# rubendhz/houdini-gsplat-renderer

Hardware: AMD Instinct MI355X
Metric: frames/sec at 1920x1080 + achieved HBM GB/s (blend kernel) (higher is better)
Workload: dtype f32

## Files before the change

houdini-gsplat-renderer_amd/csrc/gsr_device.h:

```cpp
#pragma once
#ifdef GSR_KPROF
#include <hip/hip_runtime.h>
__device__ unsigned long long g_kprof[8][16];
__device__ unsigned int g_kprof_blk[5][2][8192];
#define KPROF_BLK_BEGIN const unsigned long long kp0_ = wall_clock64();
#define KPROF_BLK_END(k, items) { if (threadIdx.x == 0 && blockIdx.x < 8192) { g_kprof_blk[k][0][blockIdx.x] = (unsigned int)(wall_clock64() - kp0_); g_kprof_blk[k][1][blockIdx.x] = (unsigned int)(items); } }
#define KPROF(k, i) { if (blockIdx.x == 0 && threadIdx.x == 0) g_kprof[k][i] = wall_clock64(); }
#define KPROFB(k, i, blk) { if (blockIdx.x == (blk) && threadIdx.x == 0) g_kprof[k][i] = wall_clock64(); }
#else
#define KPROF(k, i)
#define KPROFB(k, i, blk)
#define KPROF_BLK_BEGIN
#define KPROF_BLK_END(k, items)
#endif

#include <hip/hip_runtime.h>
#include <stdint.h>
#include "gsr_mailbox.h"

#define GSR_TILE_PX 16
#define GSR_WAVE 64

struct __attribute__((aligned(16))) GsrRecord {
    float cx, cy, hx, hy;
    float a1x, a1y, b1x, b1y;
    float r, g, b, la;
};
static_assert(sizeof(GsrRecord) == 48, "record layout");
#define GSR_KAPPA 1.2011224087864498f
#define GSR_QLIM  (2.0f * GSR_KAPPA)

struct GsrFrame {
    float ov[12];
    float pr[16];
    float vw[12];
    float ob[9];
    float io[9];
    float cam[3];
    float origin[3];
    float limx, limy;
    float sigma_vo2;
    float focal;
    float W, H;
    int32_t width, height;
    int32_t sh_order;
    int32_t tiles_x;
    int32_t tiles_y;
    int32_t shard_index, shard_count;
    int32_t shard_rpb;
    int32_t shard_first;
    int32_t local_tiles_y;
    int32_t super;
    int32_t super_shift;
    int32_t stiles_x, stiles_y;
    int32_t flags;
    uint32_t key_min, key_max;
    int32_t pyr_off[6];
    int32_t cull_dilate;
    int32_t rect_shift;
    int32_t phase;
    uint32_t idx_mask;
    float zq0, zqs;
};
typedef const GsrFrame __attribute__((address_space(4)))* GsrFrameArg;
__device__ __forceinline__ GsrFrameArg gsr_frame_arg(unsigned kernarg_off)
{
    static_assert(alignof(GsrFrame) == 4 && sizeof(GsrFrame) % 4 == 0, "the frame is a run of dwords");
    return (GsrFrameArg)((const char __attribute__((address_space(4)))*)__builtin_amdgcn_kernarg_segment_ptr() + kernarg_off);
}
__device__ __forceinline__ GsrFrame gsr_frame_fetch(GsrFrameArg p)
{
    asm volatile("" : "+s"(p));
    GsrFrame f;
    __builtin_memcpy(&f, p, sizeof(GsrFrame));
    return f;
}
#define GSR_ZQ_SHIFT 23
#define GSR_ZQ_MAX 511.0f
#define GSR_SLAB_BINS 1024
#define GSR_FLAG_NO_ALPHA_RADIUS 1
#define GSR_FLAG_NO_SAT          2
#define GSR_FLAG_FULL_KEYS       4
#define GSR_FLAG_LAZY_NO_PREFIX  8
#define GSR_FLAG_CULL_ROUNDS    16
#define GSR_FLAG_NO_DEPTH_CLASS 32
#define GSR_FLAG_NO_ZCODES      64

#ifndef BK_BUCKETS
#define BK_BUCKETS 1024
#endif
#ifndef BK_CAP
#define BK_CAP 8192
#endif
#define BK_STRIDE 64

__device__ __forceinline__ float gsr_fma(float a, float b, float c) { return __builtin_fmaf(a, b, c); }

__device__ __forceinline__ uint32_t gsr_zq(float zw, float z0, float zs)
{
    const float t = __builtin_fminf(__builtin_fmaxf((zw - z0) * zs, 0.0f), GSR_ZQ_MAX);
    return (uint32_t)t;
}

__device__ __forceinline__ float gsr_h2f(uint32_t bits16)
{
    _Float16 h = __builtin_bit_cast(_Float16, (uint16_t)bits16);
    return (float)h;
}

#define GSR_FMT_RGBA32F 0
#define GSR_FMT_RGBA16F 1
#define GSR_FMT_RGBA8   2
__host__ __device__ __forceinline__ int gsr_format_pixel_bytes(int format)
{
    return format == GSR_FMT_RGBA32F ? 16 : format == GSR_FMT_RGBA16F ? 8 : format == GSR_FMT_RGBA8 ? 4 : 0;
}
__host__ __device__ __forceinline__ uint32_t gsr_channel_half(float x)
{
    const _Float16 h = (_Float16)x;
    return (uint32_t)__builtin_bit_cast(uint16_t, h);
}
__host__ __device__ __forceinline__ uint32_t gsr_channel_unorm8(float x)
{
    float c = x > 0.0f ? x : 0.0f;
    c = c < 1.0f ? c : 1.0f;
    return (uint32_t)__builtin_fmaf(c, 255.0f, 0.5f);
}
__host__ __device__ __forceinline__ uint2 gsr_pack_rgba16f(float r, float g, float b, float a)
{
    uint2 o;
    o.x = gsr_channel_half(r) | (gsr_channel_half(g) << 16);
    o.y = gsr_channel_half(b) | (gsr_channel_half(a) << 16);
    return o;
}
__host__ __device__ __forceinline__ uint32_t gsr_pack_rgba8(float r, float g, float b, float a)
{
    return gsr_channel_unorm8(r) | (gsr_channel_unorm8(g) << 8) | (gsr_channel_unorm8(b) << 16) | (gsr_channel_unorm8(a) << 24);
}
__device__ __forceinline__ void gsr_store_packed(void* __restrict__ target, int format, size_t p, float r, float g, float b, float a)
{
    if (format == GSR_FMT_RGBA16F) reinterpret_cast<uint2*>(target)[p] = gsr_pack_rgba16f(r, g, b, a);
    else reinterpret_cast<uint32_t*>(target)[p] = gsr_pack_rgba8(r, g, b, a);
}

__host__ __device__ __forceinline__ float gsr_resolve_depth_pixel(float zsum, float cov, float cov_min)
{
    return cov >= cov_min ? __builtin_fminf(zsum / cov, 1.0f) : 1.0f;
}

#define GSR_BGK_COLOUR 1
#define GSR_BGK_IMAGE  2
__host__ __device__ __forceinline__ float4 gsr_composite_over_pixel(float4 s, float4 b)
{
    const float k = 1.0f - b.w;
    return make_float4(__builtin_fmaf(k, s.x, b.x), __builtin_fmaf(k, s.y, b.y), __builtin_fmaf(k, s.z, b.z), __builtin_fmaf(k, s.w, b.w));
}
__host__ __device__ __forceinline__ float4 gsr_background_pixel(const void* __restrict__ image, int format, size_t p)
{
    if (format == GSR_FMT_RGBA32F) return reinterpret_cast<const float4*>(image)[p];
    if (format == GSR_FMT_RGBA16F) {
        const uint2 v = reinterpret_cast<const uint2*>(image)[p];
        return make_float4((float)__builtin_bit_cast(_Float16, (uint16_t)(v.x & 0xffffu)), (float)__builtin_bit_cast(_Float16, (uint16_t)(v.x >> 16)),
                           (float)__builtin_bit_cast(_Float16, (uint16_t)(v.y & 0xffffu)), (float)__builtin_bit_cast(_Float16, (uint16_t)(v.y >> 16)));
    }
// ... 158 lines not shown
```

houdini-gsplat-renderer_amd/csrc/k_binning.h:

```cpp
#pragma once
#include "gsr_device.h"
#include "k_sort.h"

#define BN_THREADS 256
#ifndef BN_ITEMS
#define BN_ITEMS 4
#endif
#define BN_TILE (BN_THREADS * BN_ITEMS)
#define BN_WAVE_ITEMS (BN_TILE / 4)
#define BN_BINS 256

#define BN_BIG 8

__device__ __forceinline__ uint32_t bn_tile_mask(uint32_t rc, int sx, int sy, int shift)
{
    const int x0 = rc & 255, y0 = (rc >> 8) & 255, x1 = (rc >> 16) & 255, y1 = rc >> 24;
    const int e = (1 << shift) - 1;
    const int c0 = max(x0 - (sx << shift), 0), c1 = min(x1 - (sx << shift), e);
    const int r0 = max(y0 - (sy << shift), 0), r1 = min(y1 - (sy << shift), e);
    const uint32_t cols = ((2u << c1) - 1u) & ~((1u << c0) - 1u), rows = ((2u << r1) - 1u) & ~((1u << r0) - 1u);
    return cols | (rows << 16);
}

template <typename F>
__device__ __forceinline__ void bn_for_each_super(uint32_t rc, int shift, const GsrShard& sh, int stiles_x, int row_lo, int row_hi, F&& fn)
{
    const int x0 = rc & 255, y0 = (rc >> 8) & 255, x1 = (rc >> 16) & 255, y1 = rc >> 24;
    if (x1 < x0 || y1 < y0) return;
    const int sx0 = x0 >> shift, sx1 = x1 >> shift;
    for (int sy = max(y0 >> shift, row_lo); sy <= min(y1 >> shift, row_hi); ++sy) {
        if (sh.count > 1 || sh.rpb > 0) {
            const int lo = max(y0, sy << shift), hi = min(y1, ((sy + 1) << shift) - 1);
            if (gsr_owned_rect_rows(lo, hi, sh) == 0) continue;
        }
        const uint32_t rowkey = (uint32_t)sy * (uint32_t)stiles_x;
        for (int sx = sx0; sx <= sx1; ++sx) fn(rowkey + (uint32_t)sx, sx, sy);
    }
}

#ifndef BN_SPLIT_TILES
#define BN_SPLIT_TILES 16
#endif
struct BnPart { uint32_t tile; int row_lo, row_hi; };
__device__ __forceinline__ uint32_t bn_items(uint32_t nb, int rows) { const uint32_t hs = nb < (uint32_t)BN_SPLIT_TILES ? nb : (uint32_t)BN_SPLIT_TILES; return nb + hs * (uint32_t)(rows - 1); }
__device__ __forceinline__ BnPart bn_part(uint32_t v, uint32_t nb, int rows)
{
    const uint32_t hs = nb < (uint32_t)BN_SPLIT_TILES ? nb : (uint32_t)BN_SPLIT_TILES;
    if (v < hs * (uint32_t)rows) { const uint32_t t = v / (uint32_t)rows; const int r = (int)(v - t * (uint32_t)rows); return BnPart{t, r, r}; }
    return BnPart{hs + rs_tile_of_block(v - hs * (uint32_t)rows, nb - hs, true), 0, 0x7fffffff};
}

template <typename F>
__device__ __forceinline__ void bn_group_pairs(uint2 v, int shift, const GsrShard& sh, int stiles_x, int row_lo, int row_hi, F&& fn)
{
    const int lane = threadIdx.x & 63;
    const uint32_t rc = v.y;
    const int x0 = rc & 255, y0 = (rc >> 8) & 255, x1 = rc >> 16 & 255, y1 = rc >> 24;
    const bool some = x1 >= x0 && y1 >= y0;
    const int ya = max(y0 >> shift, row_lo), yb = min(y1 >> shift, row_hi);
    const int area = (some && yb >= ya) ? ((x1 >> shift) - (x0 >> shift) + 1) * (yb - ya + 1) : 0;
#ifndef BN_MANY
#define BN_MANY 6
#endif
#ifndef BN_BIG_MANY
#define BN_BIG_MANY 32
#endif
    const int thr = __builtin_popcountll(__ballot(area > BN_BIG)) > BN_MANY ? BN_BIG_MANY : BN_BIG;
    const bool big = area > thr;
    if (!big) bn_for_each_super(rc, shift, sh, stiles_x, row_lo, row_hi, [&](uint32_t d, int sx, int sy) { fn(lane, v, d, sx, sy); });
    unsigned long long bigs = __ballot(big);
    while (bigs) {
        const int L = __builtin_ctzll(bigs);
        bigs &= bigs - 1ull;
        const uint2 vL = make_uint2((uint32_t)__shfl((int)v.x, L, 64), (uint32_t)__shfl((int)v.y, L, 64));
        const uint32_t r = vL.y;
        const int X0 = r & 255, Y0 = (r >> 8) & 255, X1 = (r >> 16) & 255, Y1 = r >> 24;
        const int sx0 = X0 >> shift, sy0 = max(Y0 >> shift, row_lo);
        const int w = (X1 >> shift) - sx0 + 1, h = min(Y1 >> shift, row_hi) - sy0 + 1;
        auto cell = [&](int ry, int cx) __attribute__((always_inline)) {
            const int sy = sy0 + ry, sx = sx0 + cx;
            if (sh.count > 1 || sh.rpb > 0) {
                const int lo = max(Y0, sy << shift), hi = min(Y1, ((sy + 1) << shift) - 1);
                if (gsr_owned_rect_rows(lo, hi, sh) == 0) return;
            }
            const uint32_t dd = (uint32_t)sy * (uint32_t)stiles_x + (uint32_t)sx;
            fn(L, vL, dd, sx, sy);
        };
        if (w <= 64) {
            const int cb = w > 1 ? 32 - __builtin_clz((unsigned)(w - 1)) : 0;
            const int cx = lane & ((1 << cb) - 1), rstep = 64 >> cb;
            if (cx < w)
                for (int ry = lane >> cb; ry < h; ry += rstep) cell(ry, cx);
        } else {
            for (int t = lane; t < w * h; t += 64) { const int ry = t / w; cell(ry, t - ry * w); }
        }
    }
}

template <int ITEMS>
__global__ void __launch_bounds__(BN_THREADS)
k_bin_count(const uint2* __restrict__ sorted, const uint32_t* __restrict__ n_dev, int shift, GsrShard sh,
            int stiles_x, int stiles_y, uint32_t* __restrict__ hist, uint32_t nblk)
{
    constexpr uint32_t TILE = BN_THREADS * ITEMS;
    __shared__ uint32_t h[4][BN_BINS];
    KPROF_BLK_BEGIN
    const int wave = threadIdx.x >> 6;
    const uint32_t n = *n_dev;
    const uint32_t nb = (n + TILE - 1) / TILE;
    const uint32_t nv = bn_items(nb, stiles_y);
    for (uint32_t wi = blockIdx.x; wi < nv; wi += gridDim.x) {
        for (int b = threadIdx.x; b < 4 * BN_BINS; b += BN_THREADS) (&h[0][0])[b] = 0;
        __syncthreads();
        const BnPart part = bn_part(wi, nb, stiles_y);
        const uint32_t tile = part.tile;
        {
            const uint32_t base = tile * TILE;
#pragma unroll
            for (int k = 0; k < ITEMS; ++k) {
                const uint32_t i = base + k * BN_THREADS + threadIdx.x;
                const uint2 v = (i < n) ? sorted[i] : make_uint2(0u, GSR_RECT_EMPTY);
                bn_group_pairs(v, shift, sh, stiles_x, part.row_lo, part.row_hi,
                               [&](int, uint2, uint32_t d, int, int) { if (d < (uint32_t)BN_BINS) atomicAdd(&h[wave][d], 1u); });
            }
        }
        __syncthreads();
        const int b_lo = part.row_lo * stiles_x, b_hi = part.row_hi >= stiles_y - 1 ? BN_BINS : (part.row_hi + 1) * stiles_x;
        for (int b = b_lo + (int)threadIdx.x; b < b_hi; b += BN_THREADS)
            hist[(size_t)b * nblk + tile] = h[0][b] + h[1][b] + h[2][b] + h[3][b];
        __syncthreads();
    }
    KPROF_BLK_END(3, n < TILE ? n : TILE)
}

struct GsrRangeArgs {
    const uint32_t* totals;
    int32_t n_super;
    int32_t *sstart, *send;
    volatile unsigned long long* host_total;
    uint32_t ticket;
    unsigned long long max_pairs;
    uint32_t* redo_count;
    const uint32_t* lazy_hint;
    const uint32_t* n_sorted;
    const uint32_t* k1_counts;
    const uint32_t* sorted_keys;
    const uint32_t* depth_active;
};
__device__ __forceinline__ uint32_t bn_ranges(const GsrRangeArgs& a, bool publish, uint32_t* s_wave , unsigned long long* s_sum )
{
    if (publish && threadIdx.x == 0) {
        *a.redo_count = 0u;
        const uint32_t ns = *a.n_sorted;
        a.host_total[1] = ((unsigned long long)ns << 32) | (unsigned long long)(*a.lazy_hint & GSR_HINT_VERDICTS) |
                          (a.k1_counts[2] ? (unsigned long long)GSR_HINT_SORT_GAVE_UP : 0ull) |
                          ((a.depth_active && *a.depth_active) ? (unsigned long long)GSR_HINT_DEPTH_COVERED : 0ull);
        a.host_total[2] = (unsigned long long)a.k1_counts[1];
        a.host_total[3] = ns ? ((unsigned long long)a.sorted_keys[ns - 1u] << 32) | (unsigned long long)a.sorted_keys[0] : 0ull;
    }
    const uint32_t v = ((int)threadIdx.x < a.n_super) ? a.totals[threadIdx.x] : 0u;
    unsigned long long w = v;
#pragma unroll
    for (int d = 32; d > 0; d >>= 1) w += __shfl_down(w, d, 64);
    if ((threadIdx.x & 63) == 0) s_sum[threadIdx.x >> 6] = w;
    uint32_t tot;
    const uint32_t ex = block_excl_scan_256(v, s_wave, &tot);
    const bool too_many = s_sum[0] + s_sum[1] + s_sum[2] + s_sum[3] > a.max_pairs;
    if (publish) {
        if ((int)threadIdx.x < a.n_super) {
            a.sstart[threadIdx.x] = too_many ? 0 : (int32_t)ex;
            a.send[threadIdx.x] = too_many ? 0 : (int32_t)(ex + v);
        }
        if (threadIdx.x == 0) { *a.host_total = ((unsigned long long)a.ticket << 32) | (too_many ? (unsigned long long)GSR_MB_TOO_MANY_PAIRS : (unsigned long long)tot); __threadfence_system(); }
    }
    return too_many ? 0u : ex;
}
__global__ void __launch_bounds__(BN_BINS)
k_bin_ranges(GsrRangeArgs a)
{
    __shared__ uint32_t s_wave[4];
    __shared__ unsigned long long s_sum[4];
    (void)bn_ranges(a, true, s_wave, s_sum);
}

template <int ITEMS, bool ZQ>
__global__ void __launch_bounds__(BN_THREADS)
k_bin_place(const uint2* __restrict__ sorted, const uint32_t* __restrict__ n_dev, int shift, GsrShard sh,
            int stiles_x, int ns, const uint32_t* __restrict__ offs, const int32_t* __restrict__ sstart,
            uint32_t nblk, uint32_t cap, uint2* __restrict__ out, GsrRangeArgs ranges,
            const float* __restrict__ zwin, float zq0, float zqs)
{
    static_assert(BN_THREADS == BN_BINS, "one thread per super-tile in the range scan");
    constexpr uint32_t TILE = BN_THREADS * ITEMS;
    constexpr int NG = 4 * ITEMS;
    KPROF(0, 0)
    KPROF_BLK_BEGIN
    extern __shared__ unsigned long long bn_lds[];
    __shared__ uint32_t s_start[BN_BINS];
    __shared__ uint32_t s_rwave[4];
    __shared__ unsigned long long s_rsum[4];
    const uint32_t n = *n_dev;
    const uint32_t nb = (n + TILE - 1) / TILE;
    const bool publisher = ranges.totals && blockIdx.x == gridDim.x - 1u;
    const uint32_t workers = ranges.totals ? gridDim.x - 1u : gridDim.x;
    if (!publisher && blockIdx.x >= bn_items(nb, stiles_x > 0 ? (ns + stiles_x - 1) / stiles_x : 1)) return;
    if (ranges.totals) {
        s_start[threadIdx.x] = bn_ranges(ranges, publisher, s_rwave, s_rsum);
        if (publisher) return;
    } else {
        s_start[threadIdx.x] = ((int)threadIdx.x < ns) ? (uint32_t)sstart[threadIdx.x] : 0u;
    }
    __syncthreads();
    KPROF(0, 1)
    const int wave = threadIdx.x >> 6;
    unsigned long long* lmask = bn_lds;
    uint32_t* gpre = reinterpret_cast<uint32_t*>(bn_lds + (size_t)NG * ns);
    const int stiles_y = stiles_x > 0 ? (ns + stiles_x - 1) / stiles_x : 1;
    const uint32_t nv = bn_items(nb, stiles_y);
    for (uint32_t wi = blockIdx.x; wi < nv; wi += workers) {
    const BnPart part = bn_part(wi, nb, stiles_y);
    const uint32_t tile = part.tile;
    const uint32_t first = tile * TILE;
    KPROF(0, 2)
    for (int b = threadIdx.x; b < NG * ns; b += BN_THREADS) lmask[b] = 0ull;
    __syncthreads();
    KPROF(0, 3)
    uint2 v[ITEMS];
#pragma unroll
    for (int k = 0; k < ITEMS; ++k) {
        const int grp = k * 4 + wave;
        const uint32_t i = first + (uint32_t)grp * 64u + (threadIdx.x & 63u);
        v[k] = (i < n) ? sorted[i] : make_uint2(0u, GSR_RECT_EMPTY);
        if (ZQ && i < n) v[k].x |= gsr_zq(zwin[v[k].x], zq0, zqs) << GSR_ZQ_SHIFT;
        bn_group_pairs(v[k], shift, sh, stiles_x, part.row_lo, part.row_hi,
                       [&](int L, uint2, uint32_t d, int, int) { if (d < (uint32_t)ns) atomicOr(&lmask[grp * ns + d], 1ull << L); });
    }
    __syncthreads();
    KPROF(0, 4)
    for (int d = threadIdx.x; d < ns; d += BN_THREADS) {
        uint32_t p = s_start[d] + offs[(size_t)d * nblk + tile];
#pragma unroll
        for (int grp = 0; grp < NG; ++grp) { gpre[grp * ns + d] = p; p += (uint32_t)__builtin_popcountll(lmask[grp * ns + d]); }
    }
    __syncthreads();
    KPROF(0, 6)
#pragma unroll
    for (int k = 0; k < ITEMS; ++k) {
        const int grp = k * 4 + wave;
        bn_group_pairs(v[k], shift, sh, stiles_x, part.row_lo, part.row_hi, [&](int L, uint2 vL, uint32_t d, int sx, int sy) {
            if (d >= (uint32_t)ns) return;
            const uint32_t pos = gpre[grp * ns + d] + (uint32_t)__builtin_popcountll(lmask[grp * ns + d] & ((1ull << L) - 1ull));
            if (pos < cap) out[pos] = make_uint2(vL.x, bn_tile_mask(vL.y, sx, sy, shift));
        });
    }
    KPROF(0, 7)
    __syncthreads();
    }
    KPROF_BLK_END(0, n < TILE ? n : TILE)
}

template <typename PIX>
__global__ void __launch_bounds__(256)
k_stitch_bands(const PIX* __restrict__ gathered, int count, int rpb, int band_rows, int width, int height,
               PIX* __restrict__ out)
{
    const size_t p = (size_t)blockIdx.x * 256u + threadIdx.x;
    if (p >= (size_t)width * height) return;
    const int x = (int)(p % width), y = (int)(p / width);
    const int trow = y >> 4;
    const int g = rpb > 0 ? trow / rpb : trow % count, lrow = rpb > 0 ? trow - g * rpb : trow / count;
    const int by = lrow * GSR_TILE_PX + (y & 15);
    out[p] = gathered[((size_t)g * band_rows + by) * width + x];
}
```

houdini-gsplat-renderer_amd/csrc/k_sort.h:

```cpp
#pragma once
#include "gsr_device.h"

#define RS_THREADS 256
#ifndef RS_ITEMS
#define RS_ITEMS 12
#endif
static_assert(RS_ITEMS % 4 == 0, "k_radix_hist reads uint4");
#ifndef RS_ITEMS_MID
#define RS_ITEMS_MID 4
#endif
#define RS_TILE (RS_THREADS * RS_ITEMS)
#define RS_WAVE_ITEMS (RS_TILE / 4)
#ifndef RS_XCD_DEPTH
#define RS_XCD_DEPTH 1
#endif
#ifndef RS_XCD_BIN
#define RS_XCD_BIN 0
#endif

__device__ __forceinline__ uint32_t rs_tile_of_block(uint32_t b, uint32_t nb, bool contig)
{
    if (!contig) return b;
    const uint32_t q = nb >> 3, r = nb & 7u, x = b & 7u, i = b >> 3;
    return x * q + (x < r ? x : r) + i;
// ... 183 lines not shown
    V v_[ITEMS];
    const unsigned long long lt_mask = (1ull << lane) - 1ull;
    uint32_t gc[WAVE_BLOCKS];
    const uint32_t g_first = (tile_base + (uint32_t)wave * WAVE_ITEMS) / RS_SRC_BLOCK;
    const uint32_t g_tot = GATHER ? rs_gather_counts(src_cnt, g_first, (n + RS_SRC_BLOCK - 1) / RS_SRC_BLOCK, gc) : 0u;
#pragma unroll
    for (int r = 0; r < ITEMS; ++r) {
        const uint32_t li = wave * WAVE_ITEMS + r * 64 + lane;
        bool valid = li < nvalid;
        uint32_t key = 0xffffffffu;
        V val{};
        if (GATHER) {
            if ((uint32_t)(r * 64) >= g_tot) { k_[r] = key; v_[r] = val; meta[r] = 0xffffffffu; continue; }
            const uint32_t q = (uint32_t)(r * 64 + lane);
            valid = q < g_tot;
            if (valid) {
                const uint32_t slot = rs_gather_slot(q, g_first, gc);
                key = keys_in[slot];
                val = vals_in[slot];
            }
        } else if (valid) {
            key = keys_in[tile_base + li];
            val = vals_in[tile_base + li];
        }
        const uint32_t d = rs_digit<CLAMP>(key, shift, lo, MASK);
        unsigned long long m = __ballot(valid);
#pragma unroll
        for (int b = 0; b < DBITS; ++b) {
            const bool bit = (d >> b) & 1u;
            const unsigned long long bal = __ballot(bit);
            m &= bit ? bal : ~bal;
        }
        const uint32_t rank = (uint32_t)__builtin_popcountll(m & lt_mask);
        const uint32_t cnt = (uint32_t)__builtin_popcountll(m);
        uint32_t prev = 0;
        if (valid && rank == 0) {
            prev = wc[wave][d];
            wc[wave][d] = prev + cnt;
        }
        const int leader = m ? __builtin_ctzll(m) : 0;
        prev = __shfl(prev, leader, 64);
        k_[r] = key; v_[r] = val;
        meta[r] = valid ? (d | ((prev + rank) << DBITS)) : 0xffffffffu;
    }
    __syncthreads();
    {
        uint32_t tot_d[PER], tsum = 0;
#pragma unroll
        for (int k = 0; k < PER; ++k) {
            const int d = threadIdx.x * PER + k;
            const uint32_t c0 = wc[0][d], c1 = wc[1][d], c2 = wc[2][d], c3 = wc[3][d];
            wc[0][d] = 0; wc[1][d] = c0; wc[2][d] = c0 + c1; wc[3][d] = c0 + c1 + c2;
            tot_d[k] = c0 + c1 + c2 + c3;
            tsum += tot_d[k];
        }
        uint32_t tot;
        uint32_t ex = block_excl_scan_256(tsum, s_wave, &tot);
        if (threadIdx.x == 0) s_tile_items = tot;
#pragma unroll
        for (int k = 0; k < PER; ++k) {
            const int d = threadIdx.x * PER + k;
            dbase[d] = ex;
            gadj[d] = gadj[d] + offs[(size_t)d * nblk + tile] - ex;
            ex += tot_d[k];
        }
    }
    __syncthreads();
#pragma unroll
    for (int r = 0; r < ITEMS; ++r) {
        if (meta[r] == 0xffffffffu) continue;
        const uint32_t d = meta[r] & MASK;
        const uint32_t lp = dbase[d] + wc[wave][d] + (meta[r] >> DBITS);
        skeys[lp] = k_[r];
        svals[lp] = v_[r];
    }
    __syncthreads();
    const uint32_t tile_items = s_tile_items;
#pragma unroll
    for (int r = 0; r < ITEMS; ++r) {
        const uint32_t j = r * RS_THREADS + threadIdx.x;
        if (j < tile_items) {
            const uint32_t key = skeys[j];
            const uint32_t pos = gadj[rs_digit<CLAMP>(key, shift, lo, MASK)] + j;
            keys_out[pos] = key;
            vals_out[pos] = svals[j];
        }
    }
}

__global__ void __launch_bounds__(256)
k_pos_keys(const float4* __restrict__ geoA, uint32_t n, float cx, float cy, float cz, uint32_t key_min, uint32_t key_max,
           uint32_t* __restrict__ keys, uint32_t* __restrict__ vals)
{
    const uint32_t i = blockIdx.x * 256u + threadIdx.x;
    if (i >= n) return;
    const float4 a = geoA[i];
    const float dx = a.x - cx, dy = a.y - cy, dz = a.z - cz;
    const float d2 = __builtin_fmaf(dz, dz, __builtin_fmaf(dy, dy, dx * dx));
    uint32_t b = __builtin_bit_cast(uint32_t, d2);
    b = b < key_min ? key_min : (b > key_max ? key_max : b);
    keys[i] = b - key_min;
    vals[i] = i;
}
__global__ void __launch_bounds__(1024)
k_scan_counts(const uint32_t* __restrict__ cnt, const uint32_t* __restrict__ slots_dev, uint32_t* __restrict__ pre, uint32_t* __restrict__ n_out)
{
    __shared__ uint32_t s_w[16];
    __shared__ uint32_t s_carry;
    const uint32_t m = *slots_dev / (uint32_t)RS_SRC_BLOCK;
    const int lane = threadIdx.x & 63, wave = threadIdx.x >> 6;
    if (threadIdx.x == 0) s_carry = 0u;
    __syncthreads();
    for (uint32_t base = 0; base < m; base += 1024u) {
        const uint32_t j = base + threadIdx.x;
        const uint32_t v = j < m ? cnt[j] : 0u;
        uint32_t x = v;
#pragma unroll
        for (int d = 1; d < 64; d <<= 1) { const uint32_t y = __shfl_up(x, d, 64); if (lane >= d) x += y; }
        if (lane == 63) s_w[wave] = x;
        __syncthreads();
        uint32_t wbase = 0;
        for (int w = 0; w < wave; ++w) wbase += s_w[w];
        const uint32_t carry = s_carry;
        if (j < m) pre[j] = carry + wbase + x - v;
        __syncthreads();
        if (threadIdx.x == 1023) s_carry = carry + wbase + x;
        __syncthreads();
    }
    if (threadIdx.x == 0) *n_out = s_carry;
}
template <typename V>
__global__ void __launch_bounds__(RS_SRC_BLOCK)
k_compact_blocks(const uint32_t* __restrict__ keys_in, const V* __restrict__ vals_in, const uint32_t* __restrict__ cnt, const uint32_t* __restrict__ pre,
                 const uint32_t* __restrict__ slots_dev, uint32_t* __restrict__ keys_out, V* __restrict__ vals_out)
{
    const uint32_t k = blockIdx.x;
    if (k * (uint32_t)RS_SRC_BLOCK >= *slots_dev) return;
    if (threadIdx.x < cnt[k]) {
        const uint32_t src = k * (uint32_t)RS_SRC_BLOCK + threadIdx.x, dst = pre[k] + threadIdx.x;
        keys_out[dst] = keys_in[src];
        vals_out[dst] = vals_in[src];
    }
}

#define RL_THREADS 256
#ifndef RL_ITEMS
#define RL_ITEMS 8
#endif
#define RL_CHUNK (RL_THREADS * RL_ITEMS)
#define RL_WAVE_ITEMS (RL_CHUNK / 4)
#define RL_BINS 256
static_assert(BK_CAP >= RL_CHUNK, "a bucket's region holds at least one chunk");
#define RL_MAX_RUN 64

__device__ __forceinline__ uint32_t rl_id(uint32_t v) { return v; }
__device__ __forceinline__ uint32_t rl_id(uint2 v) { return v.x; }

template <typename V, bool GATHER>
__global__ void __launch_bounds__(RS_THREADS)
k_bucket_scatter(const uint32_t* __restrict__ keys_in, const V* __restrict__ vals_in, uint32_t n_host, const uint32_t* __restrict__ n_dev,
                 int shift, uint32_t lo, const uint32_t* __restrict__ src_cnt ,
                 uint32_t* __restrict__ gcnt , uint32_t* __restrict__ kout, V* __restrict__ vout,
                 uint32_t* __restrict__ n_out , uint32_t* __restrict__ failed)
{
    __shared__ uint32_t h[BK_BUCKETS];
    __shared__ uint32_t s_wave[4];
    const int lane = threadIdx.x & 63, wave = threadIdx.x >> 6;
    KPROF(1, 0)
    KPROF_BLK_BEGIN
    const uint32_t n = n_dev ? *n_dev : n_host;
    const uint32_t nb = (n + RS_TILE - 1) / RS_TILE;
    if (blockIdx.x >= nb) return;
    for (int b = threadIdx.x; b < BK_BUCKETS; b += RS_THREADS) h[b] = 0;
    __syncthreads();
    KPROF(1, 1)
    const uint32_t tile_base = blockIdx.x * RS_TILE;
    const uint32_t nvalid = (n - tile_base < RS_TILE) ? (n - tile_base) : RS_TILE;
    uint32_t k_[RS_ITEMS], meta[RS_ITEMS];
    static_assert(BK_BUCKETS <= 4096 && RS_TILE < (1 << 20), "meta packing");
    V v_[RS_ITEMS];
    uint32_t gc[RS_WAVE_BLOCKS];
    const uint32_t g_first = (tile_base + (uint32_t)wave * RS_WAVE_ITEMS) / RS_SRC_BLOCK;
    const uint32_t g_tot = GATHER ? rs_gather_counts(src_cnt, g_first, (n + RS_SRC_BLOCK - 1) / RS_SRC_BLOCK, gc) : 0u;
    uint32_t mine = 0;
#pragma unroll
    for (int r = 0; r < RS_ITEMS; ++r) {
        const uint32_t li = wave * RS_WAVE_ITEMS + r * 64 + lane;
        bool valid = li < nvalid;
        uint32_t key = 0u;
        V val{};
        if (GATHER) {
            const uint32_t q = (uint32_t)(r * 64 + lane);
            valid = q < g_tot;
            if (valid) { const uint32_t slot = rs_gather_slot(q, g_first, gc); key = keys_in[slot]; val = vals_in[slot]; }
        } else if (valid) {
            key = keys_in[tile_base + li]; val = vals_in[tile_base + li];
        }
        k_[r] = key; v_[r] = val; meta[r] = 0xffffffffu;
        if (valid) {
            const uint32_t d = rs_digit<true>(key, shift, lo, BK_BUCKETS - 1);
            meta[r] = d | (atomicAdd(&h[d], 1u) << 12);
            ++mine;
        }
    }
    __syncthreads();
    KPROF(1, 2)
    for (int d = threadIdx.x; d < BK_BUCKETS; d += RS_THREADS) {
        const uint32_t c = h[d];
        h[d] = c ? atomicAdd(&gcnt[(size_t)d * BK_STRIDE], c) : 0u;
    }
    if (n_out) {
        uint32_t tot;
        (void)block_excl_scan_256(mine, s_wave, &tot);
        if (threadIdx.x == 0 && tot) atomicAdd(n_out, tot);
    }
    __syncthreads();
    KPROF(1, 3)
#pragma unroll
    for (int r = 0; r < RS_ITEMS; ++r) {
        if (meta[r] == 0xffffffffu) continue;
        const uint32_t d = meta[r] & 4095u, p = h[d] + (meta[r] >> 12);
        if (p < (uint32_t)BK_CAP) { kout[(size_t)d * BK_CAP + p] = k_[r]; vout[(size_t)d * BK_CAP + p] = v_[r]; }
        else if (failed) *failed = 1u;
    }
    KPROF(1, 4)
    KPROF_BLK_END(1, mine)
}

template <typename V>
__global__ void __launch_bounds__(256)
k_bucket_scatter_k1(const uint32_t* __restrict__ keys_in, const V* __restrict__ vals_in, uint32_t n_blocks_host, const uint32_t* __restrict__ n_dev,
                    int shift, uint32_t lo, const uint32_t* __restrict__ src_cnt, uint32_t* __restrict__ gcnt,
                    uint32_t* __restrict__ kout, V* __restrict__ vout, uint32_t* __restrict__ failed,
                    const uint32_t* __restrict__ range_dev = nullptr )
{
    __shared__ uint32_t h[BK_BUCKETS];
    const int lane = threadIdx.x & 63, wave = threadIdx.x >> 6;
    if (range_dev) { lo = range_dev[0]; shift = (int)range_dev[1]; }
    uint32_t n = 0xffffffffu;
    for (uint32_t wg = blockIdx.x; wg * 4u * (uint32_t)RS_SRC_BLOCK < n; wg += gridDim.x) {
        uint32_t gb = wg * 4u + (uint32_t)wave;
        const bool surplus = gb >= n_blocks_host;
        gb = surplus ? n_blocks_host - 1u : gb;
        const uint32_t base = gb * (uint32_t)RS_SRC_BLOCK;
        const uint32_t cnt_raw = src_cnt[gb];
        uint32_t k_[4];
        V v_[4];
#pragma unroll
        for (int r = 0; r < 4; ++r) { k_[r] = keys_in[base + (uint32_t)(r * 64 + lane)]; v_[r] = vals_in[base + (uint32_t)(r * 64 + lane)]; }
        if (n == 0xffffffffu) {
            n = *n_dev;
            if (wg * 4u * (uint32_t)RS_SRC_BLOCK >= n) return;
        }
        const uint32_t cnt = (base < n && !surplus) ? cnt_raw : 0u;
        for (int b = threadIdx.x; b < BK_BUCKETS; b += 256) h[b] = 0;
        __syncthreads();
        uint32_t meta[4];
#pragma unroll
        for (int r = 0; r < 4; ++r) {
            meta[r] = 0xffffffffu;
            if ((uint32_t)(r * 64 + lane) < cnt) {
                const uint32_t d = rs_digit<true>(k_[r], shift, lo, BK_BUCKETS - 1);
                meta[r] = d | (atomicAdd(&h[d], 1u) << 12);
            }
        }
        __syncthreads();
        for (int d = threadIdx.x; d < BK_BUCKETS; d += 256) {
            const uint32_t c = h[d];
            h[d] = c ? atomicAdd(&gcnt[(size_t)d * BK_STRIDE], c) : 0u;
        }
        __syncthreads();
#pragma unroll
        for (int r = 0; r < 4; ++r) {
            if (meta[r] == 0xffffffffu) continue;
            const uint32_t d = meta[r] & 4095u, p = h[d] + (meta[r] >> 12);
            if (p < (uint32_t)BK_CAP) { kout[(size_t)d * BK_CAP + p] = k_[r]; vout[(size_t)d * BK_CAP + p] = v_[r]; }
            else if (failed) *failed = 1u;
        }
        __syncthreads();
    }
}

template <typename V>
__global__ void __launch_bounds__(RS_SRC_BLOCK)
k_bucket_scatter_direct(const uint32_t* __restrict__ keys_in, const V* __restrict__ vals_in, const uint32_t* __restrict__ n_dev,
                        int shift, uint32_t lo, const uint32_t* __restrict__ src_cnt, uint32_t* __restrict__ gcnt,
                        uint32_t* __restrict__ kout, V* __restrict__ vout, uint32_t* __restrict__ failed)
{
    const uint32_t slot = blockIdx.x * (uint32_t)RS_SRC_BLOCK + threadIdx.x;
    const uint32_t cnt = src_cnt[blockIdx.x];
    const uint32_t key = keys_in[slot];
    const V val = vals_in[slot];
    const uint32_t n = *n_dev;
    if (blockIdx.x * (uint32_t)RS_SRC_BLOCK >= n || threadIdx.x >= cnt) return;
    const uint32_t d = rs_digit<true>(key, shift, lo, BK_BUCKETS - 1);
    const uint32_t p = atomicAdd(&gcnt[(size_t)d * BK_STRIDE], 1u);
    if (p < (uint32_t)BK_CAP) { kout[(size_t)d * BK_CAP + p] = key; vout[(size_t)d * BK_CAP + p] = val; }
    else if (failed) *failed = 1u;
}

template <typename V>
__device__ __forceinline__ void rl_pass_in_lds(uint32_t (&k_)[RL_ITEMS], V (&v_)[RL_ITEMS], uint32_t n, uint32_t wq, int shift, uint32_t sub,
                                               uint32_t (*wc)[RL_BINS], uint32_t* dbase, uint32_t* dcount, uint32_t* s_wave,
                                               uint32_t* skeys, V* svals)
{
    const int lane = threadIdx.x & 63, wave = threadIdx.x >> 6;
    const unsigned long long lt_mask = (1ull << lane) - 1ull;
    for (int b = threadIdx.x; b < 4 * RL_BINS; b += RL_THREADS) (&wc[0][0])[b] = 0;
    __syncthreads();
    uint32_t meta[RL_ITEMS];
#pragma unroll
    for (int r = 0; r < RL_ITEMS; ++r) {
        const uint32_t li = (uint32_t)wave * wq + (uint32_t)r * 64u + (uint32_t)lane;
        const bool valid = (uint32_t)r * 64u < wq && li < n;
        const uint32_t d = ((k_[r] - sub) >> shift) & (RL_BINS - 1);
        unsigned long long m = __ballot(valid);
        if (m == 0ull) { meta[r] = 0xffffffffu; continue; }
#pragma unroll
        for (int b = 0; b < 8; ++b) {
            const bool bit = (d >> b) & 1u;
            const unsigned long long bal = __ballot(bit);
            m &= bit ? bal : ~bal;
        }
        const uint32_t rank = (uint32_t)__builtin_popcountll(m & lt_mask);
        const uint32_t cnt = (uint32_t)__builtin_popcountll(m);
        uint32_t prev = 0;
        if (valid && rank == 0) { prev = wc[wave][d]; wc[wave][d] = prev + cnt; }
        const int leader = m ? __builtin_ctzll(m) : 0;
        prev = __shfl(prev, leader, 64);
        meta[r] = valid ? (d | ((prev + rank) << 8)) : 0xffffffffu;
    }
    __syncthreads();
    {
        const int d = threadIdx.x;
        const uint32_t c0 = wc[0][d], c1 = wc[1][d], c2 = wc[2][d], c3 = wc[3][d];
        wc[0][d] = 0; wc[1][d] = c0; wc[2][d] = c0 + c1; wc[3][d] = c0 + c1 + c2;
        const uint32_t tot_d = c0 + c1 + c2 + c3;
        uint32_t tot;
        const uint32_t ex = block_excl_scan_256(tot_d, s_wave, &tot);
        dbase[d] = ex;
        dcount[d] = tot_d;
    }
    __syncthreads();
#pragma unroll
    for (int r = 0; r < RL_ITEMS; ++r) {
        if (meta[r] == 0xffffffffu) continue;
        const uint32_t d = meta[r] & (RL_BINS - 1);
        const uint32_t lp = dbase[d] + wc[wave][d] + (meta[r] >> 8);
        skeys[lp] = k_[r];
        svals[lp] = v_[r];
    }
    __syncthreads();
}

template <typename V>
__device__ __forceinline__ void rl_fix_ties(uint32_t* keys, V* vals, uint32_t n, uint32_t* failed)
{
    for (uint32_t j = threadIdx.x; j + 1u < n; j += RL_THREADS) {
        const uint32_t key = keys[j];
        if (keys[j + 1u] != key || (j > 0u && keys[j - 1u] == key)) continue;
        uint32_t e = j + 2u;
        while (e < n && keys[e] == key) ++e;
        if (failed && e - j > (uint32_t)RL_MAX_RUN) { *failed = 1u; continue; }
        for (uint32_t a = j + 1u; a < e; ++a) {
            const V x = vals[a];
            uint32_t b = a;
            while (b > j && rl_id(vals[b - 1u]) > rl_id(x)) { vals[b] = vals[b - 1u]; --b; }
            vals[b] = x;
        }
    }
    __syncthreads();
}

template <typename V>
__global__ void __launch_bounds__(RL_THREADS)
k_radix_local(const uint32_t* __restrict__ cnt, int low_bits, int full_bits, uint32_t lo,
              uint32_t* __restrict__ ksrc, V* __restrict__ vsrc, uint32_t* __restrict__ kdst, V* __restrict__ vdst,
              uint32_t* __restrict__ failed, uint32_t* __restrict__ n_out ,
              const uint32_t* __restrict__ range_dev = nullptr )
{
    if (range_dev) { lo = range_dev[0]; low_bits = (int)range_dev[1]; }
    __shared__ uint32_t wc[4][RL_BINS];
    __shared__ uint32_t dbase[RL_BINS], dcount[RL_BINS], gbase[RL_BINS];
    __shared__ uint32_t s_wave[4];
    __shared__ uint32_t skeys[RL_CHUNK];
    __shared__ V svals[RL_CHUNK];
    const int lane = threadIdx.x & 63, wave = threadIdx.x >> 6;
    const int b = (int)blockIdx.x;
    KPROFB(2, 0, BK_BUCKETS / 2)
    KPROF_BLK_BEGIN
    uint32_t before = 0;
    for (int d = threadIdx.x; d < b; d += RL_THREADS) { const uint32_t c = cnt[(size_t)d * BK_STRIDE]; before += c < (uint32_t)BK_CAP ? c : (uint32_t)BK_CAP; }
    uint32_t tot;
    (void)block_excl_scan_256(before, s_wave, &tot);
    const uint32_t start = tot;
    KPROFB(2, 1, BK_BUCKETS / 2)
    uint32_t n = cnt[(size_t)b * BK_STRIDE];
    n = n < (uint32_t)BK_CAP ? n : (uint32_t)BK_CAP;
    if (n_out && b == BK_BUCKETS - 1 && threadIdx.x == 0) *n_out = start + n;
    if (n == 0u) return;
    uint32_t* ks = ksrc + (size_t)b * BK_CAP;
    V* vs = vsrc + (size_t)b * BK_CAP;
    uint32_t* kd = kdst + start;
    V* vd = vdst + start;
    const bool middle = b > 0 && b < BK_BUCKETS - 1;
    const int sort_bits = middle ? low_bits : full_bits;
    const uint32_t sub = middle ? lo : 0u;
    const int npass = sort_bits <= 0 ? 0 : (sort_bits + 7) / 8;
    uint32_t k_[RL_ITEMS];
    V v_[RL_ITEMS];
    if (n <= 64u) {
        unsigned long long* packed = reinterpret_cast<unsigned long long*>(svals);
        static_assert(sizeof(V) * RL_CHUNK >= 8 * RL_THREADS, "the payload staging area holds one packed pair per thread");
        const uint32_t t = threadIdx.x;
        uint32_t key = 0u;
        V val{};
        if (t < n) { key = ks[t]; val = vs[t]; }
        const unsigned long long me = ((unsigned long long)key << 32) | (unsigned long long)rl_id(val);
        packed[t] = t < n ? me : ~0ull;
        __syncthreads();
        uint32_t rank = 0;
        for (uint32_t j0 = 0; j0 < n; j0 += 8u) {
            unsigned long long o[8];
#pragma unroll
            for (int u = 0; u < 8; ++u) o[u] = packed[j0 + (uint32_t)u];
#pragma unroll
            for (int u = 0; u < 8; ++u) rank += (o[u] < me || (o[u] == me && j0 + (uint32_t)u < t)) ? 1u : 0u;
        }
        if (t < n) { kd[rank] = key; vd[rank] = val; }
        KPROF_BLK_END(2, n)
        return;
    }
    if (n <= (uint32_t)RL_CHUNK) {
        const uint32_t wq = ((n + 255u) / 256u) * 64u;
        auto mine = [&](int r, uint32_t& li) { li = (uint32_t)wave * wq + (uint32_t)r * 64u + (uint32_t)lane; return (uint32_t)r * 64u < wq && li < n; };
#pragma unroll
        for (int r = 0; r < RL_ITEMS; ++r) {
            uint32_t li;
            k_[r] = 0u; v_[r] = V{};
            if (mine(r, li)) { k_[r] = ks[li]; v_[r] = vs[li]; }
        }
        KPROFB(2, 2, BK_BUCKETS / 2)
        if (npass == 0) {
#pragma unroll
            for (int r = 0; r < RL_ITEMS; ++r) {
                uint32_t li;
                if (mine(r, li)) { skeys[li] = k_[r]; svals[li] = v_[r]; }
            }
            __syncthreads();
        }
        for (int p = 0; p < npass; ++p) {
            rl_pass_in_lds(k_, v_, n, wq, 8 * p, sub, wc, dbase, dcount, s_wave, skeys, svals);
            if (p + 1 < npass) {
#pragma unroll
                for (int r = 0; r < RL_ITEMS; ++r) {
                    uint32_t li;
                    if (mine(r, li)) { k_[r] = skeys[li]; v_[r] = svals[li]; }
                }
                __syncthreads();
            }
        }
        KPROFB(2, 3, BK_BUCKETS / 2)
        rl_fix_ties(skeys, svals, n, failed);
        KPROFB(2, 4, BK_BUCKETS / 2)
        for (uint32_t j = threadIdx.x; j < n; j += RL_THREADS) { kd[j] = skeys[j]; vd[j] = svals[j]; }
        KPROFB(2, 5, BK_BUCKETS / 2)
        KPROF_BLK_END(2, n)
        return;
    }
    uint32_t* ka = ks; V* va = vs;
    uint32_t* kb = kd; V* vb = vd;
    for (int p = 0; p < npass; ++p) {
        const int shift = 8 * p;
        for (int d = threadIdx.x; d < 4 * RL_BINS; d += RL_THREADS) (&wc[0][0])[d] = 0;
        __syncthreads();
        for (uint32_t j = threadIdx.x; j < n; j += RL_THREADS) atomicAdd(&wc[wave][((ka[j] - sub) >> shift) & (RL_BINS - 1)], 1u);
        __syncthreads();
        {
            const int d = threadIdx.x;
            const uint32_t c = wc[0][d] + wc[1][d] + wc[2][d] + wc[3][d];
            uint32_t t2;
            gbase[d] = block_excl_scan_256(c, s_wave, &t2);
        }
        __syncthreads();
        for (uint32_t c0 = 0; c0 < n; c0 += RL_CHUNK) {
            const uint32_t m = n - c0 < (uint32_t)RL_CHUNK ? n - c0 : (uint32_t)RL_CHUNK;
#pragma unroll
            for (int r = 0; r < RL_ITEMS; ++r) {
                const uint32_t li = (uint32_t)wave * RL_WAVE_ITEMS + (uint32_t)r * 64u + (uint32_t)lane;
                k_[r] = 0u; v_[r] = V{};
                if (li < m) { k_[r] = ka[c0 + li]; v_[r] = va[c0 + li]; }
            }
            rl_pass_in_lds(k_, v_, m, (uint32_t)RL_WAVE_ITEMS, shift, sub, wc, dbase, dcount, s_wave, skeys, svals);
            for (uint32_t j = threadIdx.x; j < m; j += RL_THREADS) {
                const uint32_t key = skeys[j];
                const uint32_t d = ((key - sub) >> shift) & (RL_BINS - 1);
                const uint32_t pos = gbase[d] + (j - dbase[d]);
                kb[pos] = key;
                vb[pos] = svals[j];
            }
            __syncthreads();
            gbase[threadIdx.x] += dcount[threadIdx.x];
            __syncthreads();
        }
        __threadfence();
        __syncthreads();
        uint32_t* tk = ka; ka = kb; kb = tk;
        V* tv = va; va = vb; vb = tv;
    }
    if (ka != kd) {
        for (uint32_t j = threadIdx.x; j < n; j += RL_THREADS) { kd[j] = ka[j]; vd[j] = va[j]; }
        __threadfence();
        __syncthreads();
    }
    rl_fix_ties(kd, vd, n, failed);
    KPROF_BLK_END(2, n)
}
```

Baseline: 4587.

## Issue bucket and bin loads early to overlap global latency with setup

The bucket local-sort kernel now issues its count loads, range parameters and the first two rounds of key/value loads, before the prefix scan over bucket counts, in a striped layout. The first in-LDS radix pass is given a striped-index variant so it can consume those loads. The binning count kernel likewise loads its sorted items before zeroing the shared histogram. The aim is to hide global-memory latency behind the block scan and LDS initialisation. In exchange it raises register pressure, reads data speculatively before n is known, and changes the item-to-thread mapping for the first pass.

```diff
diff --git a/houdini-gsplat-renderer_amd/csrc/gsr_device.h b/houdini-gsplat-renderer_amd/csrc/gsr_device.h
--- a/houdini-gsplat-renderer_amd/csrc/gsr_device.h
+++ b/houdini-gsplat-renderer_amd/csrc/gsr_device.h
@@ -7,9 +7,11 @@
 #define KPROF_BLK_END(k, items) { if (threadIdx.x == 0 && blockIdx.x < 8192) { g_kprof_blk[k][0][blockIdx.x] = (unsigned int)(wall_clock64() - kp0_); g_kprof_blk[k][1][blockIdx.x] = (unsigned int)(items); } }
 #define KPROF(k, i) { if (blockIdx.x == 0 && threadIdx.x == 0) g_kprof[k][i] = wall_clock64(); }
 #define KPROFB(k, i, blk) { if (blockIdx.x == (blk) && threadIdx.x == 0) g_kprof[k][i] = wall_clock64(); }
+#define KPROFB_ARRIVED(k, i, blk) { if (blockIdx.x == (blk)) { __builtin_amdgcn_s_waitcnt(0); if (threadIdx.x == 0) g_kprof[k][i] = wall_clock64(); } }
 #else
 #define KPROF(k, i)
 #define KPROFB(k, i, blk)
+#define KPROFB_ARRIVED(k, i, blk)
 #define KPROF_BLK_BEGIN
 #define KPROF_BLK_END(k, items)
 #endif
diff --git a/houdini-gsplat-renderer_amd/csrc/k_binning.h b/houdini-gsplat-renderer_amd/csrc/k_binning.h
--- a/houdini-gsplat-renderer_amd/csrc/k_binning.h
+++ b/houdini-gsplat-renderer_amd/csrc/k_binning.h
@@ -110,16 +110,22 @@
     const uint32_t nb = (n + TILE - 1) / TILE;
     const uint32_t nv = bn_items(nb, stiles_y);
     for (uint32_t wi = blockIdx.x; wi < nv; wi += gridDim.x) {
+        const BnPart part = bn_part(wi, nb, stiles_y);
+        const uint32_t tile = part.tile;
+        uint2 vk[ITEMS];
+#pragma unroll
+        for (int k = 0; k < ITEMS; ++k) {
+            const uint32_t i = tile * TILE + k * BN_THREADS + threadIdx.x;
+            vk[k] = sorted[i < n ? i : n - 1u];
+        }
         for (int b = threadIdx.x; b < 4 * BN_BINS; b += BN_THREADS) (&h[0][0])[b] = 0;
         __syncthreads();
-        const BnPart part = bn_part(wi, nb, stiles_y);
-        const uint32_t tile = part.tile;
         {
             const uint32_t base = tile * TILE;
 #pragma unroll
             for (int k = 0; k < ITEMS; ++k) {
                 const uint32_t i = base + k * BN_THREADS + threadIdx.x;
-                const uint2 v = (i < n) ? sorted[i] : make_uint2(0u, GSR_RECT_EMPTY);
+                const uint2 v = (i < n) ? vk[k] : make_uint2(0u, GSR_RECT_EMPTY);
                 bn_group_pairs(v, shift, sh, stiles_x, part.row_lo, part.row_hi,
                                [&](int, uint2, uint32_t d, int, int) { if (d < (uint32_t)BN_BINS) atomicAdd(&h[wave][d], 1u); });
             }
diff --git a/houdini-gsplat-renderer_amd/csrc/k_sort.h b/houdini-gsplat-renderer_amd/csrc/k_sort.h
--- a/houdini-gsplat-renderer_amd/csrc/k_sort.h
+++ b/houdini-gsplat-renderer_amd/csrc/k_sort.h
@@ -359,6 +359,10 @@
 #define RL_BINS 256
 static_assert(BK_CAP >= RL_CHUNK, "a bucket's region holds at least one chunk");
 #define RL_MAX_RUN 64
+#define RL_PRE (BK_BUCKETS / RL_THREADS)
+#define RL_SPEC 2
+static_assert(BK_BUCKETS % RL_THREADS == 0, "every thread sums the same number of bucket counters");
+static_assert(RL_SPEC <= RL_ITEMS && RL_SPEC * RL_THREADS <= BK_CAP, "the rounds requested ahead of n lie inside the bucket's own region");
 
 __device__ __forceinline__ uint32_t rl_id(uint32_t v) { return v; }
 __device__ __forceinline__ uint32_t rl_id(uint2 v) { return v.x; }
@@ -506,7 +510,7 @@
     else if (failed) *failed = 1u;
 }
 
-template <typename V>
+template <typename V, bool STRIPED = false>
 __device__ __forceinline__ void rl_pass_in_lds(uint32_t (&k_)[RL_ITEMS], V (&v_)[RL_ITEMS], uint32_t n, uint32_t wq, int shift, uint32_t sub,
                                                uint32_t (*wc)[RL_BINS], uint32_t* dbase, uint32_t* dcount, uint32_t* s_wave,
                                                uint32_t* skeys, V* svals)
@@ -518,8 +522,8 @@
     uint32_t meta[RL_ITEMS];
 #pragma unroll
     for (int r = 0; r < RL_ITEMS; ++r) {
-        const uint32_t li = (uint32_t)wave * wq + (uint32_t)r * 64u + (uint32_t)lane;
-        const bool valid = (uint32_t)r * 64u < wq && li < n;
+        const uint32_t li = STRIPED ? (uint32_t)r * RL_THREADS + threadIdx.x : (uint32_t)wave * wq + (uint32_t)r * 64u + (uint32_t)lane;
+        const bool valid = (STRIPED || (uint32_t)r * 64u < wq) && li < n;
         const uint32_t d = ((k_[r] - sub) >> shift) & (RL_BINS - 1);
         unsigned long long m = __ballot(valid);
         if (m == 0ull) { meta[r] = 0xffffffffu; continue; }
@@ -586,7 +590,6 @@
               uint32_t* __restrict__ failed, uint32_t* __restrict__ n_out ,
               const uint32_t* __restrict__ range_dev = nullptr )
 {
-    if (range_dev) { lo = range_dev[0]; low_bits = (int)range_dev[1]; }
     __shared__ uint32_t wc[4][RL_BINS];
     __shared__ uint32_t dbase[RL_BINS], dcount[RL_BINS], gbase[RL_BINS];
     __shared__ uint32_t s_wave[4];
@@ -596,33 +599,51 @@
     const int b = (int)blockIdx.x;
     KPROFB(2, 0, BK_BUCKETS / 2)
     KPROF_BLK_BEGIN
+    uint32_t* ks = ksrc + (size_t)b * BK_CAP;
+    V* vs = vsrc + (size_t)b * BK_CAP;
+    uint32_t c_[RL_PRE];
+#pragma unroll
+    for (int u = 0; u < RL_PRE; ++u) {
+        const int d = (int)threadIdx.x + u * RL_THREADS;
+        c_[u] = cnt[(size_t)(d < b ? d : b) * BK_STRIDE];
+    }
+    uint32_t vzero = 0u;
+    asm volatile("" : "+v"(vzero));
+    const uint32_t n_vec = cnt[(size_t)b * BK_STRIDE + vzero];
+    const uint32_t* rd = range_dev ? range_dev : cnt;
+    const uint32_t rd_lo = rd[vzero], rd_bits = rd[1u + vzero];
+    uint32_t k_[RL_ITEMS];
+    V v_[RL_ITEMS];
+#pragma unroll
+    for (int r = 0; r < RL_SPEC; ++r) { k_[r] = ks[(uint32_t)r * RL_THREADS + threadIdx.x]; v_[r] = vs[(uint32_t)r * RL_THREADS + threadIdx.x]; }
+    KPROFB_ARRIVED(2, 1, BK_BUCKETS / 2)
     uint32_t before = 0;
-    for (int d = threadIdx.x; d < b; d += RL_THREADS) { const uint32_t c = cnt[(size_t)d * BK_STRIDE]; before += c < (uint32_t)BK_CAP ? c : (uint32_t)BK_CAP; }
+#pragma unroll
+    for (int u = 0; u < RL_PRE; ++u) {
+        const int d = (int)threadIdx.x + u * RL_THREADS;
+        before += d < b ? (c_[u] < (uint32_t)BK_CAP ? c_[u] : (uint32_t)BK_CAP) : 0u;
+    }
     uint32_t tot;
     (void)block_excl_scan_256(before, s_wave, &tot);
     const uint32_t start = tot;
-    KPROFB(2, 1, BK_BUCKETS / 2)
-    uint32_t n = cnt[(size_t)b * BK_STRIDE];
+    KPROFB(2, 2, BK_BUCKETS / 2)
+    if (range_dev) { lo = (uint32_t)__builtin_amdgcn_readfirstlane((int)rd_lo); low_bits = __builtin_amdgcn_readfirstlane((int)rd_bits); }
+    uint32_t n = (uint32_t)__builtin_amdgcn_readfirstlane((int)n_vec);
     n = n < (uint32_t)BK_CAP ? n : (uint32_t)BK_CAP;
     if (n_out && b == BK_BUCKETS - 1 && threadIdx.x == 0) *n_out = start + n;
     if (n == 0u) return;
-    uint32_t* ks = ksrc + (size_t)b * BK_CAP;
-    V* vs = vsrc + (size_t)b * BK_CAP;
     uint32_t* kd = kdst + start;
     V* vd = vdst + start;
     const bool middle = b > 0 && b < BK_BUCKETS - 1;
     const int sort_bits = middle ? low_bits : full_bits;
     const uint32_t sub = middle ? lo : 0u;
     const int npass = sort_bits <= 0 ? 0 : (sort_bits + 7) / 8;
-    uint32_t k_[RL_ITEMS];
-    V v_[RL_ITEMS];
     if (n <= 64u) {
         unsigned long long* packed = reinterpret_cast<unsigned long long*>(svals);
         static_assert(sizeof(V) * RL_CHUNK >= 8 * RL_THREADS, "the payload staging area holds one packed pair per thread");
         const uint32_t t = threadIdx.x;
-        uint32_t key = 0u;
-        V val{};
-        if (t < n) { key = ks[t]; val = vs[t]; }
+        const uint32_t key = t < n ? k_[0] : 0u;
+        const V val = t < n ? v_[0] : V{};
         const unsigned long long me = ((unsigned long long)key << 32) | (unsigned long long)rl_id(val);
         packed[t] = t < n ? me : ~0ull;
         __syncthreads();
@@ -643,21 +664,26 @@
         auto mine = [&](int r, uint32_t& li) { li = (uint32_t)wave * wq + (uint32_t)r * 64u + (uint32_t)lane; return (uint32_t)r * 64u < wq && li < n; };
 #pragma unroll
         for (int r = 0; r < RL_ITEMS; ++r) {
-            uint32_t li;
-            k_[r] = 0u; v_[r] = V{};
-            if (mine(r, li)) { k_[r] = ks[li]; v_[r] = vs[li]; }
-        }
-        KPROFB(2, 2, BK_BUCKETS / 2)
+            const uint32_t li = (uint32_t)r * RL_THREADS + threadIdx.x;
+            if (r < RL_SPEC) {
+                if (li >= n) { k_[r] = 0u; v_[r] = V{}; }
+            } else {
+                k_[r] = 0u; v_[r] = V{};
+                if (li < n) { k_[r] = ks[li]; v_[r] = vs[li]; }
+            }
+        }
+        KPROFB(2, 3, BK_BUCKETS / 2)
         if (npass == 0) {
 #pragma unroll
             for (int r = 0; r < RL_ITEMS; ++r) {
-                uint32_t li;
-                if (mine(r, li)) { skeys[li] = k_[r]; svals[li] = v_[r]; }
+                const uint32_t li = (uint32_t)r * RL_THREADS + threadIdx.x;
+                if (li < n) { skeys[li] = k_[r]; svals[li] = v_[r]; }
             }
             __syncthreads();
         }
         for (int p = 0; p < npass; ++p) {
-            rl_pass_in_lds(k_, v_, n, wq, 8 * p, sub, wc, dbase, dcount, s_wave, skeys, svals);
+            if (p == 0) rl_pass_in_lds<V, true>(k_, v_, n, wq, 0, sub, wc, dbase, dcount, s_wave, skeys, svals);
+            else rl_pass_in_lds(k_, v_, n, wq, 8 * p, sub, wc, dbase, dcount, s_wave, skeys, svals);
             if (p + 1 < npass) {
 #pragma unroll
                 for (int r = 0; r < RL_ITEMS; ++r) {
@@ -667,11 +693,11 @@
                 __syncthreads();
             }
         }
-        KPROFB(2, 3, BK_BUCKETS / 2)
+        KPROFB(2, 4, BK_BUCKETS / 2)
         rl_fix_ties(skeys, svals, n, failed);
-        KPROFB(2, 4, BK_BUCKETS / 2)
+        KPROFB(2, 5, BK_BUCKETS / 2)
         for (uint32_t j = threadIdx.x; j < n; j += RL_THREADS) { kd[j] = skeys[j]; vd[j] = svals[j]; }
-        KPROFB(2, 5, BK_BUCKETS / 2)
+        KPROFB(2, 6, BK_BUCKETS / 2)
         KPROF_BLK_END(2, n)
         return;
     }
```

After: 4549. No clear change (-0.8%).
